# nanoporetech/scrappie

Hardware: AMD Instinct MI355X
Metric: raw samples/sec, rgrgr_r94 4k-sample reads (higher is better)
Workload: dtype f32 (3xf16 split products, 22-bit operands, fp32 accumulate)

## Files before the change

### scrappie_amd/csrc/sh_decode_teams.h

```cpp
#ifndef SH_DECODE_TEAMS_H
#define SH_DECODE_TEAMS_H

#ifndef SH_FVT_WBUF
#define SH_FVT_WBUF 3
#endif
#ifndef SH_FVT_PROD_PRIO
#define SH_FVT_PROD_PRIO 1
#endif
#ifndef SH_FVT_ABL
#define SH_FVT_ABL 0
#endif
#ifndef SH_FVT_FLIP
#define SH_FVT_FLIP 3
#endif
#ifndef SH_FVT_STAMP
#ifdef SH_EXPERIMENTS
#define SH_FVT_STAMP 1
#else
#define SH_FVT_STAMP 0
#endif
#endif
#define SH_FVT_NTH 768
#define SH_FVT_LDS_FLOATS (1024 * 16 + 64 * 256 + 2 * 64 * 16 + 2 * 2 * 8 * 16 + 4 * 9 * 16 + 65 * 16 + 2 * 3 * 512 + 3 * 2 * 4 * 4)

template <bool SKIP0, bool DIV, bool NOCLAMP = false>
__global__ __launch_bounds__(SH_FVT_NTH) void k_ff_viterbi_teams(ShFfArgs f, ShVitArgs a, ShMeta md) {
    static_assert(!(DIV && NOCLAMP), "with temperatures the clamp stays");
    constexpr int NCW = 8, NPW = 4, PPT = 8, NQ = 256, NH = 1024, KS = 3, KQ = 6, TPP = 16, HT = 8, NG = 9, WB = SH_FVT_WBUF;
    static_assert(SH_SUM_GROUP == HT, "half a pass of a producer is one row-sum group");
    static_assert(WB >= 2 && WB <= 4, "weight ring");
    extern __shared__ __attribute__((aligned(16))) float smem[];
    float *sc = smem;
    float *ring = sc + NH * 16;
    float *skk = ring + 64 * 256;
    float *redv = skk + 2 * 64 * 16;
    int *redi = (int *)(redv + 2 * NCW * 16);
    float *gsum = (float *)(redi + 2 * NCW * 16);
    float *sBias = gsum + 4 * NG * 16;
    unsigned *xp = (unsigned *)(sBias + 65 * 16);
    unsigned *sStay = xp + 2 * KS * 512;

    const int tid = threadIdx.x, lane = tid & 63, b = lane & 15, q = lane >> 4;
    const int wave = __builtin_amdgcn_readfirstlane(tid >> 6);
    const bool decoder = wave < NCW;
    const float mp = a.min_prob, mpm1 = 1.0f - a.min_prob;
    const float lbound = (mp > 0.0f) ? 1.0e-3f - __logf(mp) : INFINITY;
    unsigned long long vA = 0, vB = 0, vC = 0, vD = 0, vt0 = 0, vt1 = 0;
    (void)vt0; (void)vt1;
#undef VSTAMP
#if SH_FVT_STAMP
#define VSTAMP(acc) do { if (a.dbg) { vt1 = __builtin_readcyclecounter(); acc += vt1 - vt0; vt0 = vt1; } } while (0)
#else
#define VSTAMP(acc) do { } while (0)
#endif

    if (tid < KS * 2 * 4 * 4) sStay[tid] = f.wpiece[(long long)(64) * KS * 512 + (tid >> 4) * 256 + ((tid >> 2) & 3) * 64 + (tid & 3)];
    for (int j = tid; j < 65 * 16; j += SH_FVT_NTH) sBias[j] = f.bfrag[((j >> 4) * 64 + ((j >> 2) & 3) * 16) * 4 + (j & 3)];

    int tile = blockIdx.x, s0 = 0, s1 = -1, ord = 0;
    if (a.seg) { const ShGruSegD sg = a.seg[blockIdx.x]; tile = sg.tile; s0 = sg.s0; s1 = sg.s1; ord = sg.pad; }
    tile = __builtin_amdgcn_readfirstlane(tile); s0 = __builtin_amdgcn_readfirstlane(s0); s1 = __builtin_amdgcn_readfirstlane(s1);
    const int Tt = __builtin_amdgcn_readfirstlane(md.tile_T[tile]);
    if (s1 < 0) s1 = Tt;
    const long long boff = __builtin_amdgcn_readfirstlane((int)md.tile_boff[tile]);
    const int rd = tile * 16 + b;
    int myT = md.rT[rd];
    asm volatile("" : "+v"(myT));
    const long long hpo = a.hp_side ? a.hp_off[rd] : 0;
    float pstart = 0.0f, pend = -SH_BIG;

    const int cw = decoder ? wave : 0;
    float *myq = sc + cw * 256 + lane * 4;
    const float *mye = ring + cw * 512 + lane * 4;
    const float *mysrc = sc + cw * 64 + b * 4 + q;
#define SH_FVT_MT(i) (16 * ((i) >> 1) + 8 * ((i) & 1))

    if (s0 == 0) {
        if (decoder) {
#pragma unroll
            for (int i = 0; i < PPT; i++) *(f32x4 *)(myq + SH_FVT_MT(i) * 256) = (f32x4){-SH_BIG, -SH_BIG, -SH_BIG, -SH_BIG};
            if (lane < 16) { redv[wave * 16 + b] = -SH_BIG - a.local_pen; redi[wave * 16 + b] = 4 * wave; }
        }
    } else {
        if (tid == 0) {
            if (!sh_wait_flag(a.flag + tile, (unsigned)ord, a.err)) __hip_atomic_store(a.err, 1u, __ATOMIC_RELAXED, __HIP_MEMORY_SCOPE_AGENT);
        }
        __syncthreads();
        __builtin_amdgcn_fence(__ATOMIC_ACQUIRE, "agent");
        if (decoder) {
            const float *vst = a.vstate + (long long)tile * (NH * 16 + 32);
            float bv = -INFINITY;
            int bi = 0x7fffffff;
#pragma unroll
            for (int i = 0; i < PPT; i++) {
                const int Q = 4 * (SH_FVT_MT(i) + cw) + q;
                const f32x4 pv = *(const f32x4 *)(vst + (Q * 16 + b) * 4);
                *(f32x4 *)(myq + SH_FVT_MT(i) * 256) = pv;
                {
                    const float ve = __builtin_fmaxf(__builtin_fmaxf(pv[0], pv[1]), __builtin_fmaxf(pv[2], pv[3])) - a.local_pen;
                    bi = (ve > bv) ? Q : bi;
                    bv = __builtin_fmaxf(bv, ve);
                }
            }
            pstart = vst[NH * 16 + b];
            pend = vst[NH * 16 + 16 + b];
            float ov = __shfl_xor(bv, 16); int oi = __shfl_xor(bi, 16);
            argmax_merge(bv, bi, ov, oi);
            ov = __shfl_xor(bv, 32); oi = __shfl_xor(bi, 32);
            argmax_merge(bv, bi, ov, oi);
            if (lane < 16) { redv[wave * 16 + b] = bv; redi[wave * 16 + b] = bi; }
        }
    }

    if (!decoder) {
        const int pw = wave - NCW;
#if SH_FVT_PROD_PRIO
        __builtin_amdgcn_s_setprio(SH_FVT_PROD_PRIO);
#endif
        const unsigned *wmine = f.wpiece + (long long)(TPP * pw) * KS * 512;
        ShSplit W[WB][KS];
        const unsigned lofs = (unsigned)lane * 4u;
        typedef const __attribute__((address_space(1))) unsigned *gu32;
        typedef const __attribute__((address_space(1))) u32x4 *gu32x4;
        gu32 wp = (gu32)wmine;
        auto w_load = [&](int k) {
            static_assert(KS == 3, "two bases per tile: immediate offsets reach 4095 bytes");
            gu32 b0 = wp, b1 = wp + 1024;
            asm volatile("" : "+s"(b0), "+s"(b1));
            W[(k % HT) % WB][0].p1 = __builtin_bit_cast(f16x8, *(gu32x4)(b0 + lofs));
            W[(k % HT) % WB][0].p2 = __builtin_bit_cast(f16x8, *(gu32x4)(b0 + 256 + lofs));
            W[(k % HT) % WB][1].p1 = __builtin_bit_cast(f16x8, *(gu32x4)(b0 + 512 + lofs));
            W[(k % HT) % WB][1].p2 = __builtin_bit_cast(f16x8, *(gu32x4)(b0 + 768 + lofs));
            W[(k % HT) % WB][2].p1 = __builtin_bit_cast(f16x8, *(gu32x4)(b1 + lofs));
            W[(k % HT) % WB][2].p2 = __builtin_bit_cast(f16x8, *(gu32x4)(b1 + 256 + lofs));
            wp = (k == TPP - 1) ? (gu32)wmine : wp + KS * 512;
            asm volatile("" : "+s"(wp));
        };
        auto w_prime = [&](int k0) {
#pragma unroll
            for (int k = 0; k < WB - 1; k++) w_load(k0 + k);
        };
        const int xks = pw < KS ? pw : KS - 1;
        f32x4 xr[2][2];
        auto xraw_load = [&](int u) {
#pragma unroll
            for (int j = 0; j < 2; j++) {
                const float *p = f.in + ((boff + min(u + j, s1 - 1)) * KQ + 2 * xks) * 256;
                xr[j][0] = *(const f32x4 *)(p + lofs);
                xr[j][1] = *(const f32x4 *)(p + 256 + lofs);
            }
        };
        auto xp_publish = [&]() {
            if (pw < KS) {
#pragma unroll
                for (int j = 0; j < 2; j++) {
                    f32x4 v0 = xr[j][0], v1 = xr[j][1];
                    if (DIV) { v0 = v0 / f.in_div; v1 = v1 / f.in_div; }
                    const ShSplit sp = split8(v0, v1);
                    unsigned *d = xp + (j * KS + pw) * 512 + lane * 4;
                    *(u32x4 *)d = __builtin_bit_cast(u32x4, sp.p1);
                    *(u32x4 *)(d + 256) = __builtin_bit_cast(u32x4, sp.p2);
                }
            }
        };
        auto e_of = [&](float acc) { return DIV ? d_exp((acc * SH_OINV) / f.out_div) : NOCLAMP ? d_exp_acc_inrange(acc) : d_exp_acc(acc); };
        auto group_out = [&](float part, int u, int g) {
            const float v = rows_sum(part);
            if (lane < 16) gsum[((u & 3) * NG + g) * 16 + b] = v;
        };
        float *myring = ring + (TPP * pw) * 256 + lane * 4;
        auto s1_half = [&](auto Hc, int u) {
            constexpr int H = decltype(Hc)::value;
#if defined(SH_FVT_DBG_ROLE) && SH_FVT_DBG_ROLE == 1
            return;
#endif
            const float *mybias = sBias + (TPP * pw + HT * H) * 16 + 4 * q;
            ShSplit bp[2][KS];
#pragma unroll
            for (int j = 0; j < 2; j++)
#pragma unroll
                for (int ks = 0; ks < KS; ks++) bp[j][ks] = load_pieces(xp + (j * KS + ks) * 512, lane);
            float part0 = 0.0f, part1 = 0.0f;
            auto tile_out = [&](int k, const f32x4 &acc0, const f32x4 &acc1) {
                f32x4 ex0, ex1;
#pragma unroll
                for (int r = 0; r < 4; r++) { ex0[r] = e_of(acc0[r]); ex1[r] = e_of(acc1[r]); }
                part0 += (ex0[0] + ex0[1]) + (ex0[2] + ex0[3]);
                part1 += (ex1[0] + ex1[1]) + (ex1[2] + ex1[3]);
                if (SH_FVT_ABL & 8) {
#pragma unroll
                    for (int r = 0; r < 4; r++) { ex0[r] = fin_log(ex0[r], mpm1, mp); ex1[r] = fin_log(ex1[r], mpm1, mp); }
                }
                *(f32x4 *)(myring + (2 * k) * 256) = ex0;
                *(f32x4 *)(myring + (2 * k + 1) * 256) = ex1;
            };
#pragma unroll
            for (int k = 0; k < HT; k++) {
                f32x4 acc0 = *(const f32x4 *)(mybias + k * 16), acc1 = acc0;
                if (k + WB - 1 < HT) w_load(HT * H + k + WB - 1);
                const ShSplit (&A)[KS] = W[k % WB];
#pragma unroll
                for (int ks = 0; ks < KS; ks++) { acc0 = mfma16(A[ks].p1, bp[0][ks].p2, acc0); acc1 = mfma16(A[ks].p1, bp[1][ks].p2, acc1); }
#pragma unroll
                for (int ks = 0; ks < KS; ks++) { acc0 = mfma16(A[ks].p2, bp[0][ks].p1, acc0); acc1 = mfma16(A[ks].p2, bp[1][ks].p1, acc1); }
#pragma unroll
                for (int ks = 0; ks < KS; ks++) { acc0 = mfma16(A[ks].p1, bp[0][ks].p1, acc0); acc1 = mfma16(A[ks].p1, bp[1][ks].p1, acc1); }
                tile_out(k, acc0, acc1);
                __builtin_amdgcn_sched_barrier(0);
            }
            group_out(part0, u, 2 * pw + H);
            group_out(part1, u + 1, 2 * pw + H);
            if (H == 1 && pw == NPW - 1) {
                ShSplit Ws[KS];
#pragma unroll
                for (int ks = 0; ks < KS; ks++) {
                    const u32x4 a1 = *(const u32x4 *)(sStay + ((ks * 2 + 0) * 4 + q) * 4), a2 = *(const u32x4 *)(sStay + ((ks * 2 + 1) * 4 + q) * 4);
                    const u32x4 z = {0u, 0u, 0u, 0u};
                    Ws[ks].p1 = __builtin_bit_cast(f16x8, b == 0 ? a1 : z);
                    Ws[ks].p2 = __builtin_bit_cast(f16x8, b == 0 ? a2 : z);
                }
#pragma unroll
                for (int j = 0; j < 2; j++) {
                    f32x4 acc = *(const f32x4 *)(sBias + 64 * 16 + 4 * q);
                    acc = split_dot<KS>(Ws, bp[j], acc);
                    f32x4 ex;
#pragma unroll
                    for (int r = 0; r < 4; r++) ex[r] = (4 * q + r < 1) ? e_of(acc[r]) : 0.0f;
                    group_out((ex[0] + ex[1]) + (ex[2] + ex[3]), u + j, NG - 1);
                }
            }
        };
        const std::integral_constant<int, 0> H0{};
        const std::integral_constant<int, 1> H1{};

        const bool any = s1 > s0;
        if (any) xraw_load(s0);
        __syncthreads();
        if (any) { xp_publish(); w_prime(0); }
        lds_barrier();
        if (any) s1_half(H0, s0);
        lds_barrier();
        if (any) w_prime(HT);
        lds_barrier();
        if (any) { s1_half(H1, s0); __builtin_amdgcn_sched_barrier(0); xraw_load(s0 + 2); }
        lds_barrier();
        if (a.dbg) vt0 = __builtin_readcyclecounter();
        for (int t = s0; t < s1; t += 2) {
            const bool more = (t + 2 < s1) && !(SH_FVT_ABL & 1);
            if (more) { xp_publish(); w_prime(0); }
            VSTAMP(vA);
            lds_barrier();
            VSTAMP(vB);
            if (more) s1_half(H0, t + 2);
            VSTAMP(vC);
            lds_barrier();
            VSTAMP(vD);
            if (more) w_prime(HT);
            VSTAMP(vA);
            lds_barrier();
            VSTAMP(vB);
            if (more) s1_half(H1, t + 2);
            __builtin_amdgcn_sched_barrier(0);
            xraw_load(t + 4);
            VSTAMP(vC);
            lds_barrier();
            VSTAMP(vD);
        }
        __syncthreads();
        if (s1 >= Tt) __syncthreads();
        if (a.dbg && lane == 0) { unsigned long long *d = a.dbg + ((long long)blockIdx.x * 12 + wave) * 8; d[0] = vA; d[1] = vB; d[2] = vC; d[3] = vD; d[4] = (unsigned long long)(s1 - s0); }
        return;
    }
    {
        f32x4 eN[2][PPT];
        auto drain = [&](auto a0, auto s0c, auto a1, auto s1c) {
            constexpr int A0 = decltype(a0)::value, S0 = decltype(s0c)::value, A1 = decltype(a1)::value, S1 = decltype(s1c)::value;
#pragma unroll
            for (int rl = 0; rl < PPT / 2; rl++) { eN[A0][2 * rl + S0] = *(const f32x4 *)(mye + rl * 4096); eN[A1][2 * rl + S1] = *(const f32x4 *)(mye + rl * 4096 + 256); }
        };
        const std::integral_constant<int, 0> I0{};
        const std::integral_constant<int, 1> I1{};
        __syncthreads();
        lds_barrier();
        lds_barrier();
        drain(I0, I0, I1, I0);
        lds_barrier();
        lds_barrier();
        if (a.dbg) vt0 = __builtin_readcyclecounter();
        const unsigned tofs = (unsigned)lane;
        auto block = [&](const int t, auto first_c) {
            constexpr bool FIRST = decltype(first_c)::value;
            const f32x4 (&e)[PPT] = eN[FIRST ? 0 : 1];
            const long long cb = boff + t;
            constexpr int par = FIRST ? 0 : 1;
#if defined(SH_FVT_DBG_ROLE) && SH_FVT_DBG_ROLE == 2
            lds_barrier(); lds_barrier(); return;
#endif
            if (!FIRST && t >= s1) {
                drain(I0, I0, I0, I1);
                lds_barrier(); lds_barrier();
                return;
            }

            float sv[PPT];
            int sr[PPT];
#pragma unroll
            for (int i = 0; i < PPT; i++) {
                float v = mysrc[SH_FVT_MT(i) * 64];
                int ri = 0;
                if (!(SH_FVT_ABL & 2)) {
#pragma unroll
                    for (int r = 1; r < 4; r++) {
                        const float c = mysrc[(r * 64 + SH_FVT_MT(i)) * 64];
                        const bool up = v < c;
                        v = up ? c : v;
                        ri = up ? r : ri;
                    }
                }
                sv[i] = v; sr[i] = ri;
                if (i == PPT / 2 - 1) __builtin_amdgcn_sched_barrier(0);
            }
#pragma unroll
            for (int c = 0; c < 2; c++) {
                float v = sv[c];
                int ri = 4 * sr[c];
                if (!(SH_FVT_ABL & 2)) {
#pragma unroll
                    for (int rl = 1; rl < 4; rl++) argmax_merge(v, ri, sv[2 * rl + c], 4 * sr[2 * rl + c] + rl);
                }
                *(f32x2 *)(skk + ((32 * c + 4 * cw + q) * 16 + b) * 2) = (f32x2){v, __builtin_bit_cast(float, ri)};
            }
            unsigned srp = 0;
#pragma unroll
            for (int i = 0; i < PPT; i++) srp |= (unsigned)sr[i] << (2 * i);
            float ev = 0.f; int tbe_in = 0;
            if (cw == 0) {
                int ei;
                typedef __attribute__((address_space(3))) const float *ldsf;
                ldsf rv = (ldsf)(redv + b);
                asm volatile("" : "+v"(rv));
                ev = rv[par * NCW * 16];
                ei = __builtin_bit_cast(int, rv[(2 + par) * NCW * 16]);
#pragma unroll
                for (int w = 1; w < NCW; w++) {
                    const float ov = rv[(par * NCW + w) * 16], oif = rv[((2 + par) * NCW + w) * 16];
                    argmax_merge(ev, ei, ov, __builtin_bit_cast(int, oif));
                }
                const f32x4 q4 = *(const f32x4 *)(sc + ((ei & (NQ - 1)) * 16 + b) * 4);
                int e0 = 3;
                e0 = (q4[2] - a.local_pen == ev) ? 2 : e0;
                e0 = (q4[1] - a.local_pen == ev) ? 1 : e0;
                e0 = (q4[0] - a.local_pen == ev) ? 0 : e0;
                tbe_in = 4 * ei + e0;
            }
            __builtin_amdgcn_sched_barrier(0);
            if (FIRST) drain(I0, I1, I1, I1);
            else drain(I0, I0, I0, I1);
            VSTAMP(vA);
            lds_barrier();
            VSTAMP(vB);

            float tot = 0.0f;
#pragma unroll
            for (int w = 0; w < NG; w++) tot += gsum[((t & 3) * NG + w) * 16 + b];
            const float rmf = d_rcp(tot) * mpm1;
            const float stay_lp = fin_log(gsum[((t & 3) * NG + NG - 1) * 16 + b], rmf, mp);
            const bool active = t < myT;
            const unsigned long long actmask = __builtin_amdgcn_ballot_w64(active);
            if (a.hp_side && active && tid < 16) (a.hp_side + (hpo + t) * 5)[4] = stay_lp;
            const float rm = active ? rmf : 0.0f;
            const float mpx = active ? mp : 0.0f;
            const float stay_v = active ? stay_lp - a.stay_pen : 0.0f;
            const float stay_act = stay_lp - a.stay_pen;
            const float hold = fmaxf(-a.local_pen, stay_act);
            const float nstart = pstart + hold;
            if (cw == 0) {
                float nend = pend + hold;
                const bool enter_end = ev > nend;
                nend = enter_end ? ev : nend;
                if (active && tid < 16) a.tb_end[cb * 16 + b] = enter_end ? tbe_in : NH + 1;
                if (active) pend = nend;
            }
            float bv = -INFINITY;
            int bi = 0x7fffffff;
            f32x4 pv_n; f32x2 kk_n;
            auto q_fetch = [&](int i) {
                pv_n = *(const f32x4 *)(myq + SH_FVT_MT(i) * 256);
                kk_n = *(const f32x2 *)(skk + ((SH_FVT_MT(i) + cw) * 16 + b) * 2);
            };
            q_fetch(0);
            float hpv[4] = {0.f, 0.f, 0.f, 0.f};
#pragma unroll
            for (int i = 0; i < PPT; i++) {
                const int QB = 4 * (SH_FVT_MT(i) + cw);
                const int Q = QB + q;
                const f32x4 pv = pv_n;
                const float kv = kk_n[0];
                const float krf = kk_n[1];
                const int kr = __builtin_bit_cast(int, krf);
                if (i + 1 < PPT) q_fetch(i + 1);
                f32x4 l4;
#pragma unroll
                for (int k = 0; k < 4; k++) l4[k] = (SH_FVT_ABL & 24) ? e[i][k] : fin_log(e[i][k], rm, mpx);
#pragma unroll
                for (int k = 0; k < 4; k++) {
                    const int s = k * ((NH - 1) / 3), sq = s >> 2;
                    if (i == 2 * (sq >> 6) + ((sq >> 5) & 1)) hpv[k] = l4[s & 3];
                }
                const float svi = sv[i];
                const unsigned cstep = SH_TB_STEP + ((srp >> (2 * i)) & 3u), cskip = SH_TB_SKIP + (unsigned)kr;
                const unsigned cstart = SH_TB_START;
                unsigned codes = 0;
                f32x4 ns;
#define SH_FVT_STATE(E)                                                                                         \
                {                                                                                               \
                    float s_ = pv[E] + stay_v;                                                  \
                    const float st = l4[E] + svi;                                           \
                    SH_CODE_LT(E, codes, s_, st, cstep);                                                        \
                    s_ = __builtin_fmaxf(s_, st);                                                               \
                    const float sk = SKIP0 ? l4[E] + kv : (l4[E] + kv) - a.skip_pen;        \
                    SH_CODE_LT(E, codes, s_, sk, cskip);                                                        \
                    s_ = __builtin_fmaxf(s_, sk);                                                               \
                    const float fs = pstart + l4[E];                                  \
                    SH_CODE_LT(E, codes, s_, fs, cstart);                                                       \
                    s_ = __builtin_fmaxf(s_, fs);                                                               \
                    ns[E] = s_;                                                                                 \
                }
                bool fast = false;
                float m = 0.f;
                unsigned cm = cstart;
                if (SKIP0) {
                    m = __builtin_fmaxf(__builtin_fmaxf(svi, kv), pstart);
                    const float md = __builtin_amdgcn_fmed3f(svi, kv, pstart);
                    const unsigned long long unclear = __builtin_amdgcn_fcmpf(m - md, (lbound + __builtin_fabsf(m)) * SH_FVT_GAP, 13 );
                    fast = (unclear & actmask) == 0;
                    cm = (kv == m) ? cskip : cm;
                    cm = (svi == m) ? cstep : cm;
                }
                if (fast) {
#define SH_FVT_FAST(E)                                                                                          \
                    {                                                                                           \
                        const float s_ = pv[E] + stay_v;                                        \
                        const float mv = l4[E] + m;                           \
                        SH_CODE_LT(E, codes, s_, mv, cm);                                                       \
                        ns[E] = __builtin_fmaxf(s_, mv);                                                        \
                    }
                    SH_FVT_FAST(0) SH_FVT_FAST(1) SH_FVT_FAST(2) SH_FVT_FAST(3)
#undef SH_FVT_FAST
                } else { SH_FVT_STATE(0) SH_FVT_STATE(1) SH_FVT_STATE(2) SH_FVT_STATE(3) }
#undef SH_FVT_STATE
                *(f32x4 *)(myq + SH_FVT_MT(i) * 256) = ns;
                if (!(SH_FVT_ABL & 4)) (a.tb + (cb * NQ + QB) * 16)[tofs] = codes;
                else asm volatile("" :: "v"(codes));
                {
                    const float ve = d_max4(ns) - a.local_pen;
                    bi = (ve > bv) ? Q : bi;
                    bv = __builtin_fmaxf(bv, ve);
                }
                __builtin_amdgcn_sched_barrier(0);
#if SH_FVT_FLIP
                if (cw >= 4) { if (i == PPT - 1) __builtin_amdgcn_s_setprio(1); else if (i == SH_FVT_FLIP - 1) __builtin_amdgcn_s_setprio(0); }
#endif
            }
            if (active) pstart = nstart;
            if (a.hp_side && active) {
#pragma unroll
                for (int k = 0; k < 4; k++) {
                    const int sq = (k * ((NH - 1) / 3)) >> 2;
                    if (cw == ((sq >> 2) & 7) && q == (sq & 3)) (a.hp_side + (hpo + t) * 5)[k] = hpv[k];
                }
            }
            {
                rows_argmax(bv, bi);
                if (lane < 16) { redv[((par ^ 1) * NCW + wave) * 16 + b] = bv; redi[((par ^ 1) * NCW + wave) * 16 + b] = bi; }
            }
            VSTAMP(vC);
            lds_barrier();
            VSTAMP(vD);
        };
        for (int t = s0; t < s1; t += 2) {
            block(t, std::true_type{});
            block(t + 1, std::false_type{});
#pragma unroll
            for (int rl = 0; rl < PPT / 2; rl++) eN[1][2 * rl] = eN[0][2 * rl + 1];
        }
    }

    if (s1 < Tt) {
        if (decoder) {
            float *vst = a.vstate + (long long)tile * (NH * 16 + 32);
#pragma unroll
            for (int i = 0; i < PPT; i++) {
                const int Q = 4 * (SH_FVT_MT(i) + cw) + q;
                *(f32x4 *)(vst + (Q * 16 + b) * 4) = *(const f32x4 *)(myq + SH_FVT_MT(i) * 256);
            }
            if (tid < 16) { vst[NH * 16 + b] = pstart; vst[NH * 16 + 16 + b] = pend; }
        }
        __builtin_amdgcn_fence(__ATOMIC_RELEASE, "agent");
        __syncthreads();
        if (tid == 0) __hip_atomic_store(a.flag + tile, (unsigned)ord + 1u, __ATOMIC_RELEASE, __HIP_MEMORY_SCOPE_AGENT);
    } else {
        float bv = -INFINITY;
        int bi = 0x7fffffff;
        if (decoder) {
#pragma unroll
            for (int i = 0; i < PPT; i++) {
                const int Q = 4 * (SH_FVT_MT(i) + cw) + q;
                const f32x4 pv = *(const f32x4 *)(myq + SH_FVT_MT(i) * 256);
#pragma unroll
                for (int k = 0; k < 4; k++) argmax_merge(bv, bi, pv[k], 4 * Q + k);
            }
            float ov = __shfl_xor(bv, 16); int oi = __shfl_xor(bi, 16);
            argmax_merge(bv, bi, ov, oi);
            ov = __shfl_xor(bv, 32); oi = __shfl_xor(bi, 32);
            argmax_merge(bv, bi, ov, oi);
        }
        __syncthreads();
        if (decoder && lane < 16) { redv[wave * 16 + b] = bv; redi[wave * 16 + b] = bi; }
        __syncthreads();
        if (tid < 16) {
            float ev = redv[b]; int ei = redi[b];
            for (int w = 1; w < NCW; w++) argmax_merge(ev, ei, redv[w * 16 + b], redi[w * 16 + b]);
            if (pstart > ev) { ev = pstart; ei = NH; }
            if (pend > ev) { ev = pend; ei = NH + 1; }
            a.final_state[rd] = ei;
            a.final_score[rd] = ev;
        }
        if (a.dump_final && a.vstate && decoder) {
            float *vst = a.vstate + (long long)tile * (NH * 16 + 32);
#pragma unroll
            for (int i = 0; i < PPT; i++) {
                const int Q = 4 * (SH_FVT_MT(i) + cw) + q;
                *(f32x4 *)(vst + (Q * 16 + b) * 4) = *(const f32x4 *)(myq + SH_FVT_MT(i) * 256);
            }
            if (tid < 16) { vst[NH * 16 + b] = pstart; vst[NH * 16 + 16 + b] = pend; }
        }
    }
    if (a.dbg && lane == 0) { unsigned long long *d = a.dbg + ((long long)blockIdx.x * 12 + wave) * 8; d[0] = vA; d[1] = vB; d[2] = vC; d[3] = vD; d[4] = (unsigned long long)(s1 - s0); }
#undef VSTAMP
#undef SH_FVT_MT
}

#endif
```

Before: 1.583 billion.

## Reduce per-row end argmax via LDS atomic max on packed keys

Replaces the per-wave store of end-state argmax plus a serial merge over eight waves by wave 0 with a 64-bit LDS atomic max on an order-preserving (value, ~index) key, so wave 0 reads one slot and resets it. It also precomputes the skip and step traceback codes with their offsets folded in (3-bit step packing), fuses the gap threshold into an fma, and initialises the first code with a compare/cndmask instead of zero plus OR. Traceback stores use SGPR base pointers with immediate offsets. The atomic path adds LDS atomic contention and depends on tie-breaking matching the old argmax_merge ordering.

```diff
diff --git a/scrappie_amd/csrc/sh_decode_teams.h b/scrappie_amd/csrc/sh_decode_teams.h
--- a/scrappie_amd/csrc/sh_decode_teams.h
+++ b/scrappie_amd/csrc/sh_decode_teams.h
@@ -20,6 +20,17 @@
 #define SH_FVT_STAMP 0
 #endif
 #endif
+__device__ __forceinline__ unsigned long long end_key(float v, int i) {
+    const unsigned u = __builtin_bit_cast(unsigned, v);
+    const unsigned hi = u ^ ((unsigned)((int)u >> 31) | 0x80000000u);
+    return ((unsigned long long)hi << 32) | (unsigned)~i;
+}
+__device__ __forceinline__ void end_unkey(unsigned long long k, float &v, int &i) {
+    const unsigned hi = (unsigned)(k >> 32);
+    v = __builtin_bit_cast(float, hi ^ (~(unsigned)((int)hi >> 31) | 0x80000000u));
+    i = (int)~(unsigned)k;
+}
+
 #define SH_FVT_NTH 768
 #define SH_FVT_LDS_FLOATS (1024 * 16 + 64 * 256 + 2 * 64 * 16 + 2 * 2 * 8 * 16 + 4 * 9 * 16 + 65 * 16 + 2 * 3 * 512 + 3 * 2 * 4 * 4)
 
@@ -35,6 +46,8 @@
     float *skk = ring + 64 * 256;
     float *redv = skk + 2 * 64 * 16;
     int *redi = (int *)(redv + 2 * NCW * 16);
+    typedef __attribute__((address_space(3))) unsigned long long *ldsk;
+    ldsk redk = (ldsk)redv;
     float *gsum = (float *)(redi + 2 * NCW * 16);
     float *sBias = gsum + 4 * NG * 16;
     unsigned *xp = (unsigned *)(sBias + 65 * 16);
@@ -45,6 +58,7 @@
     const bool decoder = wave < NCW;
     const float mp = a.min_prob, mpm1 = 1.0f - a.min_prob;
     const float lbound = (mp > 0.0f) ? 1.0e-3f - __logf(mp) : INFINITY;
+    const float lbgap = lbound * SH_FVT_GAP;
     unsigned long long vA = 0, vB = 0, vC = 0, vD = 0, vt0 = 0, vt1 = 0;
     (void)vt0; (void)vt1;
 #undef VSTAMP
@@ -79,9 +93,10 @@
         if (decoder) {
 #pragma unroll
             for (int i = 0; i < PPT; i++) *(f32x4 *)(myq + SH_FVT_MT(i) * 256) = (f32x4){-SH_BIG, -SH_BIG, -SH_BIG, -SH_BIG};
-            if (lane < 16) { redv[wave * 16 + b] = -SH_BIG - a.local_pen; redi[wave * 16 + b] = 4 * wave; }
+            if (wave == 0 && lane < 16) { redk[b] = end_key(-SH_BIG - a.local_pen, 0); redk[16 + b] = 0; }
         }
     } else {
+        if (tid < 32) redk[tid] = 0;
         if (tid == 0) {
             if (!sh_wait_flag(a.flag + tile, (unsigned)ord, a.err)) __hip_atomic_store(a.err, 1u, __ATOMIC_RELAXED, __HIP_MEMORY_SCOPE_AGENT);
         }
@@ -108,7 +123,7 @@
             argmax_merge(bv, bi, ov, oi);
             ov = __shfl_xor(bv, 32); oi = __shfl_xor(bi, 32);
             argmax_merge(bv, bi, ov, oi);
-            if (lane < 16) { redv[wave * 16 + b] = bv; redi[wave * 16 + b] = bi; }
+            if (lane < 16) __hip_atomic_fetch_max(redk + b, end_key(bv, bi), __ATOMIC_RELAXED, __HIP_MEMORY_SCOPE_WORKGROUP);
         }
     }
 
@@ -307,14 +322,14 @@
 #pragma unroll
             for (int i = 0; i < PPT; i++) {
                 float v = mysrc[SH_FVT_MT(i) * 64];
-                int ri = 0;
+                int ri = (int)SH_TB_STEP;
                 if (!(SH_FVT_ABL & 2)) {
 #pragma unroll
                     for (int r = 1; r < 4; r++) {
                         const float c = mysrc[(r * 64 + SH_FVT_MT(i)) * 64];
                         const bool up = v < c;
                         v = up ? c : v;
-                        ri = up ? r : ri;
+                        ri = up ? (int)SH_TB_STEP + r : ri;
                     }
                 }
                 sv[i] = v; sr[i] = ri;
@@ -322,30 +337,24 @@
             }
 #pragma unroll
             for (int c = 0; c < 2; c++) {
+                constexpr int KOFS = (int)SH_TB_SKIP - 4 * (int)SH_TB_STEP;
                 float v = sv[c];
-                int ri = 4 * sr[c];
+                int ri = 4 * sr[c] + KOFS;
                 if (!(SH_FVT_ABL & 2)) {
 #pragma unroll
-                    for (int rl = 1; rl < 4; rl++) argmax_merge(v, ri, sv[2 * rl + c], 4 * sr[2 * rl + c] + rl);
+                    for (int rl = 1; rl < 4; rl++) argmax_merge(v, ri, sv[2 * rl + c], 4 * sr[2 * rl + c] + (rl + KOFS));
                 }
                 *(f32x2 *)(skk + ((32 * c + 4 * cw + q) * 16 + b) * 2) = (f32x2){v, __builtin_bit_cast(float, ri)};
             }
+            static_assert(SH_TB_STEP + 3u < 8u, "a step code in three bits");
             unsigned srp = 0;
 #pragma unroll
-            for (int i = 0; i < PPT; i++) srp |= (unsigned)sr[i] << (2 * i);
+            for (int i = 0; i < PPT; i++) srp |= (unsigned)sr[i] << (3 * i);
             float ev = 0.f; int tbe_in = 0;
             if (cw == 0) {
                 int ei;
-                typedef __attribute__((address_space(3))) const float *ldsf;
-                ldsf rv = (ldsf)(redv + b);
-                asm volatile("" : "+v"(rv));
-                ev = rv[par * NCW * 16];
-                ei = __builtin_bit_cast(int, rv[(2 + par) * NCW * 16]);
-#pragma unroll
-                for (int w = 1; w < NCW; w++) {
-                    const float ov = rv[(par * NCW + w) * 16], oif = rv[((2 + par) * NCW + w) * 16];
-                    argmax_merge(ev, ei, ov, __builtin_bit_cast(int, oif));
-                }
+                end_unkey(redk[par * 16 + b], ev, ei);
+                redk[par * 16 + b] = 0;
                 const f32x4 q4 = *(const f32x4 *)(sc + ((ei & (NQ - 1)) * 16 + b) * 4);
                 int e0 = 3;
                 e0 = (q4[2] - a.local_pen == ev) ? 2 : e0;
@@ -383,6 +392,9 @@
             }
             float bv = -INFINITY;
             int bi = 0x7fffffff;
+            typedef __attribute__((address_space(1))) unsigned *gtb;
+            gtb tb0 = (gtb)a.tb + ((cb * NQ + 4 * cw) * 16 + 1024), tb1 = tb0 + 2048;
+            asm volatile("" : "+s"(tb0), "+s"(tb1));
             f32x4 pv_n; f32x2 kk_n;
             auto q_fetch = [&](int i) {
                 pv_n = *(const f32x4 *)(myq + SH_FVT_MT(i) * 256);
@@ -397,7 +409,7 @@
                 const f32x4 pv = pv_n;
                 const float kv = kk_n[0];
                 const float krf = kk_n[1];
-                const int kr = __builtin_bit_cast(int, krf);
+                const unsigned cskip = __builtin_bit_cast(unsigned, krf);
                 if (i + 1 < PPT) q_fetch(i + 1);
                 f32x4 l4;
 #pragma unroll
@@ -408,15 +420,19 @@
                     if (i == 2 * (sq >> 6) + ((sq >> 5) & 1)) hpv[k] = l4[s & 3];
                 }
                 const float svi = sv[i];
-                const unsigned cstep = SH_TB_STEP + ((srp >> (2 * i)) & 3u), cskip = SH_TB_SKIP + (unsigned)kr;
+                const unsigned cstep = (srp >> (3 * i)) & 7u;
                 const unsigned cstart = SH_TB_START;
-                unsigned codes = 0;
+                unsigned codes;
                 f32x4 ns;
-#define SH_FVT_STATE(E)                                                                                         \
+                static_assert(SH_TB_STAY == 0u && SH_TB_STEP + 3u < 256u && SH_TB_SKIP + 15u < 256u && SH_TB_START < 256u,
+                              "SH_FVT_LT_FIRST copies all 32 bits of x (cstep, cskip, cstart or cm): every code register is zero above its low byte");
+#define SH_FVT_LT_FIRST(E, codes, a, b, x)                                                                      \
+                asm("v_cmp_lt_f32 vcc, %1, %2\n\tv_cndmask_b32 %0, 0, %3, vcc" : "=v"(codes) : "v"(a), "v"(b), "v"(x) : "vcc")
+#define SH_FVT_STATE(E, LT1)                                                                                    \
                 {                                                                                               \
                     float s_ = pv[E] + stay_v;                                                  \
                     const float st = l4[E] + svi;                                           \
-                    SH_CODE_LT(E, codes, s_, st, cstep);                                                        \
+                    LT1(E, codes, s_, st, cstep);                                                               \
                     s_ = __builtin_fmaxf(s_, st);                                                               \
                     const float sk = SKIP0 ? l4[E] + kv : (l4[E] + kv) - a.skip_pen;        \
                     SH_CODE_LT(E, codes, s_, sk, cskip);                                                        \
@@ -432,25 +448,29 @@
                 if (SKIP0) {
                     m = __builtin_fmaxf(__builtin_fmaxf(svi, kv), pstart);
                     const float md = __builtin_amdgcn_fmed3f(svi, kv, pstart);
-                    const unsigned long long unclear = __builtin_amdgcn_fcmpf(m - md, (lbound + __builtin_fabsf(m)) * SH_FVT_GAP, 13 );
+                    static_assert(SH_FVT_GAP == 4.76837158203125e-07f, "the fused threshold needs a power of two");
+                    const unsigned long long unclear = __builtin_amdgcn_fcmpf(m - md, __builtin_fmaf(__builtin_fabsf(m), SH_FVT_GAP, lbgap), 13 );
                     fast = (unclear & actmask) == 0;
                     cm = (kv == m) ? cskip : cm;
                     cm = (svi == m) ? cstep : cm;
                 }
-                if (fast) {
-#define SH_FVT_FAST(E)                                                                                          \
+                if (__builtin_expect(fast, true)) {
+#define SH_FVT_FAST(E, LT1)                                                                                    \
                     {                                                                                           \
                         const float s_ = pv[E] + stay_v;                                        \
                         const float mv = l4[E] + m;                           \
-                        SH_CODE_LT(E, codes, s_, mv, cm);                                                       \
+                        LT1(E, codes, s_, mv, cm);                                                              \
                         ns[E] = __builtin_fmaxf(s_, mv);                                                        \
                     }
-                    SH_FVT_FAST(0) SH_FVT_FAST(1) SH_FVT_FAST(2) SH_FVT_FAST(3)
+                    SH_FVT_FAST(0, SH_FVT_LT_FIRST) SH_FVT_FAST(1, SH_CODE_LT) SH_FVT_FAST(2, SH_CODE_LT) SH_FVT_FAST(3, SH_CODE_LT)
 #undef SH_FVT_FAST
-                } else { SH_FVT_STATE(0) SH_FVT_STATE(1) SH_FVT_STATE(2) SH_FVT_STATE(3) }
+                } else { SH_FVT_STATE(0, SH_FVT_LT_FIRST) SH_FVT_STATE(1, SH_CODE_LT) SH_FVT_STATE(2, SH_CODE_LT) SH_FVT_STATE(3, SH_CODE_LT) }
 #undef SH_FVT_STATE
+#undef SH_FVT_LT_FIRST
                 *(f32x4 *)(myq + SH_FVT_MT(i) * 256) = ns;
-                if (!(SH_FVT_ABL & 4)) (a.tb + (cb * NQ + QB) * 16)[tofs] = codes;
+                gtb tbq = i < PPT / 2 ? tb0 : tb1;
+                asm volatile("" : "+s"(tbq));
+                if (!(SH_FVT_ABL & 4)) (tbq + (512 * (i % (PPT / 2)) - 1024))[tofs] = codes;
                 else asm volatile("" :: "v"(codes));
                 {
                     const float ve = d_max4(ns) - a.local_pen;
@@ -472,7 +492,7 @@
             }
             {
                 rows_argmax(bv, bi);
-                if (lane < 16) { redv[((par ^ 1) * NCW + wave) * 16 + b] = bv; redi[((par ^ 1) * NCW + wave) * 16 + b] = bi; }
+                if (lane < 16) __hip_atomic_fetch_max(redk + ((par ^ 1) * 16 + b), end_key(bv, bi), __ATOMIC_RELAXED, __HIP_MEMORY_SCOPE_WORKGROUP);
             }
             VSTAMP(vC);
             lds_barrier();
```

Result: faster. 1.600 billion (median of 6 runs) (+1.1%).
